# cbacary/MoDeGPT

Hardware: AMD Instinct MI355X
Metric: transformer layers compressed/sec (covariance+decomp+rebuild), Llama-3-8B @30% (higher is better)
Workload: dtype f64 from int8 MFMA digit planes, exact route: nine plane pairs + fp64 remainder sums, nothing truncated (error <= 5e-15 per call: fp64 rounding)

## Files before the change

modegpt_amd/csrc/mlp.hip:

```cpp
#include "common.hpp"

namespace mdg {
int gemm_f64(int64_t M, int64_t N, int64_t K, double alpha, const void* A, int a_dtype, int64_t sa_i, int64_t sa_k,
             const int64_t* a_rows, const void* B, int b_dtype, int64_t sb_k, int64_t sb_j, double beta, void* C,
             int c_dtype, int64_t ldc, int64_t batch, int64_t a_bs, int64_t b_bs, int64_t c_bs, int flags,
             hipStream_t st);
int potrf_lower(double* A, int64_t n, int64_t lda, double* inv_diag, hipStream_t st);
int potrs_lower(const double* L, int64_t n, int64_t ldl, const double* inv_diag, double* X, int64_t nrhs, int64_t ldx,
                double* ws, hipStream_t st);
size_t potrs_ws_elems(int64_t n, int64_t nrhs);
int copy_lower(const double* src, int64_t ld_src, const int64_t* idx, double* dst, int64_t ldd, int64_t n,
               double ridge, hipStream_t st);
}

using namespace mdg;

static int64_t ckk_pitch(int64_t r) { return (r + 15) / 16 * 16; }
extern "C" size_t mdg_nystrom_down_ws_bytes(int64_t n, int64_t r, int64_t d) {
  return ((size_t)r * ckk_pitch(r) + mdg_potrf_inv_diag_elems(r) + (size_t)r * d + potrs_ws_elems(r, d)) * sizeof(double);
}

static int nystrom_down(const double* C, int64_t n, int64_t ldc, const int64_t* idx, int64_t r, const void* Wd, int64_t d, int64_t ld_wd,
                        int w_dtype, double eps, void* down_out, int64_t ld_out, double* down_f64, void* ws, size_t ws_bytes,
                        void* side_stream, void* ev_fork, void* ev_join, void* stream);

extern "C" int mdg_nystrom_down(const double* C, int64_t n, int64_t ldc, const int64_t* idx, int64_t r, const void* Wd,
                                int64_t d, int64_t ld_wd, int w_dtype, double eps, void* down_out, int64_t ld_out,
                                double* down_f64, void* ws, size_t ws_bytes, void* stream) {
  return nystrom_down(C, n, ldc, idx, r, Wd, d, ld_wd, w_dtype, eps, down_out, ld_out, down_f64, ws, ws_bytes, nullptr, nullptr, nullptr, stream);
}

extern "C" int mdg_nystrom_down_overlapped(const double* C, int64_t n, int64_t ldc, const int64_t* idx, int64_t r, const void* Wd,
                                           int64_t d, int64_t ld_wd, int w_dtype, double eps, void* down_out, int64_t ld_out,
                                           double* down_f64, void* ws, size_t ws_bytes, void* side_stream, void* ev_fork, void* ev_join,
                                           void* stream) {
  MDG_CLEAR();
  MDG_CHECK_ARG(side_stream && ev_fork && ev_join && side_stream != stream,
                "mdg_nystrom_down_overlapped: needs a second stream and two events of the caller's");
  return nystrom_down(C, n, ldc, idx, r, Wd, d, ld_wd, w_dtype, eps, down_out, ld_out, down_f64, ws, ws_bytes, side_stream, ev_fork, ev_join, stream);
}

static int nystrom_down(const double* C, int64_t n, int64_t ldc, const int64_t* idx, int64_t r, const void* Wd, int64_t d, int64_t ld_wd,
                        int w_dtype, double eps, void* down_out, int64_t ld_out, double* down_f64, void* ws, size_t ws_bytes,
                        void* side_stream, void* ev_fork, void* ev_join, void* stream) {
  MDG_CLEAR();
  MDG_CHECK_ARG(C && idx && Wd && down_out, "mdg_nystrom_down: null pointer");
  MDG_CHECK_ARG(w_dtype == MDG_BF16 || w_dtype == MDG_F64, "mdg_nystrom_down: W_d must be bf16 or f64 (got %d)", w_dtype);
  MDG_CHECK_ARG(n > 0 && r > 0 && r <= n && d > 0 && ldc >= n && ld_wd >= n && ld_out >= r,
                "mdg_nystrom_down: bad sizes (n=%lld r=%lld d=%lld)", (long long)n, (long long)r, (long long)d);
  MDG_CHECK_ARG(ws && ws_bytes >= mdg_nystrom_down_ws_bytes(n, r, d), "mdg_nystrom_down: workspace %zu < required %zu",
                ws_bytes, mdg_nystrom_down_ws_bytes(n, r, d));
  hipStream_t st = (hipStream_t)stream;
  double* Ckk = (double*)ws;
  const int64_t ldk = ckk_pitch(r);
  double* inv = Ckk + (size_t)r * ldk;
  double* X = inv + mdg_potrf_inv_diag_elems(r);
  double* solve_ws = X + (size_t)r * d;
  MDG_TRY(copy_lower(C, ldc, idx, Ckk, ldk, r, eps, st));
  hipStream_t cross_st = st;
  if (side_stream) {
    cross_st = (hipStream_t)side_stream;
    MDG_HIP(hipEventRecord((hipEvent_t)ev_fork, st));
    MDG_HIP(hipStreamWaitEvent(cross_st, (hipEvent_t)ev_fork, 0));
  }
  MDG_TRY(gemm_f64(r, d, n, 1.0, C, MDG_F64, ldc, 1, idx, Wd, w_dtype, 1, ld_wd, 0.0, X, MDG_F64, d, 1, 0, 0, 0, 0, cross_st));
  if (side_stream) MDG_HIP(hipEventRecord((hipEvent_t)ev_join, cross_st));
  const int rc_potrf = potrf_lower(Ckk, r, ldk, inv, st);
  if (side_stream) MDG_HIP(hipStreamWaitEvent(st, (hipEvent_t)ev_join, 0));
  if (rc_potrf != MDG_OK) return rc_potrf;
  MDG_TRY(potrs_lower(Ckk, r, ldk, inv, X, d, d, solve_ws, st));
  if (down_f64) MDG_HIP(hipMemcpyAsync(down_f64, X, (size_t)r * d * sizeof(double), hipMemcpyDeviceToDevice, st));
  return mdg_cast_transpose_f64_bf16(X, r, d, d, down_out, ld_out, stream);
}
```

Baseline: 1.170.

## Shrink Nystrom down-projection GEMM to complement columns via algebraic identity

The down-projection GEMM over all n columns is replaced by an identity. Because the selected columns' block is the ridge-shifted Ckk, the solution equals W_S plus a Cholesky solve of a GEMM over only the n−r unselected columns, minus the ridge term. New kernels build the complement index list, compact C and W_d into padded dense buffers, and seed the right-hand side with the -eps·W_S correction. A fused add-cast-transpose kernel adds W_S back and replaces the separate memcpy and cast. The cost is extra workspace, a single-block scan kernel and compaction passes, plus slightly different fp64 rounding in the rebuilt weights.

```diff
diff --git a/modegpt_amd/csrc/mlp.hip b/modegpt_amd/csrc/mlp.hip
--- a/modegpt_amd/csrc/mlp.hip
+++ b/modegpt_amd/csrc/mlp.hip
@@ -16,8 +16,97 @@
 using namespace mdg;
 
 static int64_t ckk_pitch(int64_t r) { return (r + 15) / 16 * 16; }
+static int64_t comp_pitch(int64_t n, int64_t r) { return (n - r + BK - 1) / BK * BK; }
+static size_t solve_part_bytes(int64_t r, int64_t d) {
+  return ((size_t)r * ckk_pitch(r) + mdg_potrf_inv_diag_elems(r) + (size_t)r * d + potrs_ws_elems(r, d)) * sizeof(double);
+}
 extern "C" size_t mdg_nystrom_down_ws_bytes(int64_t n, int64_t r, int64_t d) {
-  return ((size_t)r * ckk_pitch(r) + mdg_potrf_inv_diag_elems(r) + (size_t)r * d + potrs_ws_elems(r, d)) * sizeof(double);
+  const size_t Kp = (size_t)comp_pitch(n, r);
+  return align_up(solve_part_bytes(r, d), 16) + 16 + align_up((size_t)r * Kp * 8, 16) + align_up((size_t)d * Kp * 8, 16) +
+         align_up((size_t)(n - r) * 8, 16) + align_up((size_t)n * 4, 16);
+}
+
+namespace mdg {
+
+__device__ __forceinline__ int64_t clamp_index(int64_t i, int64_t n) { return i < 0 ? 0 : (i >= n ? n - 1 : i); }
+
+__global__ __launch_bounds__(1024) void complement_kernel(const int64_t* idx, int64_t r, int64_t n, int64_t K, int* marks, int64_t* comp) {
+  __shared__ int sums[1024];
+  const int tid = threadIdx.x;
+  for (int64_t i = tid; i < n; i += 1024) marks[i] = 0;
+  __syncthreads();
+  for (int64_t p = tid; p < r; p += 1024) {
+    const int64_t i = idx[p];
+    if (i >= 0 && i < n) marks[i] = 1;
+  }
+  __syncthreads();
+  const int64_t per = (n + 1023) / 1024;
+  const int64_t b = min((int64_t)tid * per, n), e = min(b + per, n);
+  int c = 0;
+  for (int64_t i = b; i < e; i++) c += marks[i] ? 0 : 1;
+  sums[tid] = c;
+  __syncthreads();
+  for (int o = 1; o < 1024; o <<= 1) {
+    int v = tid >= o ? sums[tid - o] : 0;
+    __syncthreads();
+    sums[tid] += v;
+    __syncthreads();
+  }
+  int64_t pos = sums[tid] - c;
+  for (int64_t i = b; i < e && pos < K; i++)
+    if (!marks[i]) comp[pos++] = i;
+}
+
+template <typename T>
+__global__ __launch_bounds__(256) void compact_cols_kernel(const T* src, int64_t ld_src, const int64_t* rows, int64_t n, const int64_t* comp,
+                                                           int64_t K, int64_t Kp, T* dst) {
+  const int64_t p = blockIdx.x;
+  const T* s = src + (rows ? clamp_index(rows[p], n) : p) * ld_src;
+  T* o = dst + p * Kp;
+  for (int64_t q = threadIdx.x; q < Kp; q += 256) o[q] = q < K ? s[comp[q]] : (T)0;
+}
+
+template <int DT>
+__global__ __launch_bounds__(256) void ridge_rhs_kernel(const double* C, int64_t n, int64_t ldc, const int64_t* idx, int64_t r, const void* Wd,
+                                                        int64_t d, int64_t ld_wd, double eps, double* X) {
+  __shared__ double t[32][33];
+  const int tx = threadIdx.x & 31, ty = threadIdx.x >> 5;
+  const int64_t p0 = (int64_t)blockIdx.y * 32, j0 = (int64_t)blockIdx.x * 32;
+  const int64_t col = p0 + tx < r ? clamp_index(idx[p0 + tx], n) : -1;
+  double eps_p = 0.;
+  if (col >= 0) {
+    const double c = C[col * ldc + col];
+    eps_p = (c + eps) - c;
+  }
+  for (int j = ty; j < 32; j += 8)
+    if (col >= 0 && j0 + j < d) t[j][tx] = -(eps_p * load_f64<DT>(Wd, (j0 + j) * ld_wd + col));
+  __syncthreads();
+  for (int p = ty; p < 32; p += 8)
+    if (p0 + p < r && j0 + tx < d) X[(p0 + p) * d + j0 + tx] = t[tx][p];
+}
+
+template <int DT>
+__global__ __launch_bounds__(256) void add_cast_transpose_kernel(const double* X, const int64_t* idx, int64_t r, int64_t n, const void* Wd,
+                                                                 int64_t d, int64_t ld_wd, bf16_t* out, int64_t ld_out, double* f64_out) {
+  __shared__ double t[32][33];
+  const int tx = threadIdx.x & 31, ty = threadIdx.x >> 5;
+  const int64_t p0 = (int64_t)blockIdx.y * 32, j0 = (int64_t)blockIdx.x * 32;
+  for (int p = ty; p < 32; p += 8)
+    t[p][tx] = (p0 + p < r && j0 + tx < d) ? X[(p0 + p) * d + j0 + tx] : 0.;
+  __syncthreads();
+  const int64_t col = p0 + tx < r ? clamp_index(idx[p0 + tx], n) : -1;
+  for (int j = ty; j < 32; j += 8)
+    if (col >= 0 && j0 + j < d) {
+      const double v = load_f64<DT>(Wd, (j0 + j) * ld_wd + col) + t[tx][j];
+      out[(j0 + j) * ld_out + p0 + tx] = f64_to_bf16(v);
+      t[tx][j] = v;
+    }
+  if (!f64_out) return;
+  __syncthreads();
+  for (int p = ty; p < 32; p += 8)
+    if (p0 + p < r && j0 + tx < d) f64_out[(p0 + p) * d + j0 + tx] = t[p][tx];
+}
+
 }
 
 static int nystrom_down(const double* C, int64_t n, int64_t ldc, const int64_t* idx, int64_t r, const void* Wd, int64_t d, int64_t ld_wd,
@@ -56,6 +145,15 @@
   double* inv = Ckk + (size_t)r * ldk;
   double* X = inv + mdg_potrf_inv_diag_elems(r);
   double* solve_ws = X + (size_t)r * d;
+  const int64_t K = n - r, Kp = comp_pitch(n, r);
+  char* tail = (char*)align_up((size_t)((uintptr_t)ws + solve_part_bytes(r, d)), 16);
+  double* Cbar = (double*)tail;
+  void* Wbar = tail + align_up((size_t)r * Kp * 8, 16);
+  int64_t* comp = (int64_t*)((char*)Wbar + align_up((size_t)d * Kp * 8, 16));
+  int* marks = (int*)((char*)comp + align_up((size_t)K * 8, 16));
+  const bool w_bf16 = w_dtype == MDG_BF16;
+  dim3 tiles((unsigned)ceil_div(d, 32), (unsigned)ceil_div(r, 32));
+  MDG_CHECK_ARG(tiles.y < 65536 && d < (1ll << 31), "mdg_nystrom_down: too many rows");
   MDG_TRY(copy_lower(C, ldc, idx, Ckk, ldk, r, eps, st));
   hipStream_t cross_st = st;
   if (side_stream) {
@@ -63,12 +161,32 @@
     MDG_HIP(hipEventRecord((hipEvent_t)ev_fork, st));
     MDG_HIP(hipStreamWaitEvent(cross_st, (hipEvent_t)ev_fork, 0));
   }
-  MDG_TRY(gemm_f64(r, d, n, 1.0, C, MDG_F64, ldc, 1, idx, Wd, w_dtype, 1, ld_wd, 0.0, X, MDG_F64, d, 1, 0, 0, 0, 0, cross_st));
+  if (w_bf16) hipLaunchKernelGGL(ridge_rhs_kernel<MDG_BF16>, tiles, dim3(256), 0, cross_st, C, n, ldc, idx, r, Wd, d, ld_wd, eps, X);
+  else hipLaunchKernelGGL(ridge_rhs_kernel<MDG_F64>, tiles, dim3(256), 0, cross_st, C, n, ldc, idx, r, Wd, d, ld_wd, eps, X);
+  MDG_LAUNCH_CHECK();
+  if (K > 0) {
+    hipLaunchKernelGGL(complement_kernel, dim3(1), dim3(1024), 0, cross_st, idx, r, n, K, marks, comp);
+    MDG_LAUNCH_CHECK();
+    hipLaunchKernelGGL(compact_cols_kernel<double>, dim3((unsigned)r), dim3(256), 0, cross_st, C, ldc, idx, n, comp, K, Kp, Cbar);
+    MDG_LAUNCH_CHECK();
+    if (w_bf16)
+      hipLaunchKernelGGL(compact_cols_kernel<bf16_t>, dim3((unsigned)d), dim3(256), 0, cross_st, (const bf16_t*)Wd, ld_wd, (const int64_t*)nullptr,
+                         n, comp, K, Kp, (bf16_t*)Wbar);
+    else
+      hipLaunchKernelGGL(compact_cols_kernel<double>, dim3((unsigned)d), dim3(256), 0, cross_st, (const double*)Wd, ld_wd, (const int64_t*)nullptr,
+                         n, comp, K, Kp, (double*)Wbar);
+    MDG_LAUNCH_CHECK();
+    MDG_TRY(gemm_f64(r, d, Kp, 1.0, Cbar, MDG_F64, Kp, 1, nullptr, Wbar, w_dtype, 1, Kp, 1.0, X, MDG_F64, d, 1, 0, 0, 0, 0, cross_st));
+  }
   if (side_stream) MDG_HIP(hipEventRecord((hipEvent_t)ev_join, cross_st));
   const int rc_potrf = potrf_lower(Ckk, r, ldk, inv, st);
   if (side_stream) MDG_HIP(hipStreamWaitEvent(st, (hipEvent_t)ev_join, 0));
   if (rc_potrf != MDG_OK) return rc_potrf;
   MDG_TRY(potrs_lower(Ckk, r, ldk, inv, X, d, d, solve_ws, st));
-  if (down_f64) MDG_HIP(hipMemcpyAsync(down_f64, X, (size_t)r * d * sizeof(double), hipMemcpyDeviceToDevice, st));
-  return mdg_cast_transpose_f64_bf16(X, r, d, d, down_out, ld_out, stream);
+  if (w_bf16)
+    hipLaunchKernelGGL(add_cast_transpose_kernel<MDG_BF16>, tiles, dim3(256), 0, st, X, idx, r, n, Wd, d, ld_wd, (bf16_t*)down_out, ld_out, down_f64);
+  else
+    hipLaunchKernelGGL(add_cast_transpose_kernel<MDG_F64>, tiles, dim3(256), 0, st, X, idx, r, n, Wd, d, ld_wd, (bf16_t*)down_out, ld_out, down_f64);
+  MDG_LAUNCH_CHECK();
+  return MDG_OK;
 }
```

New measurement: 1.186, median of 6. 1.01x the previous value.
